# 0xPabloxx/3d-pointcloud-orientation-estimation

Hardware: AMD Instinct MI355X
Metric: clouds/sec fwd+bwd, pointnet_pp_vonMises N=1024 (higher is better)
Workload: dtype f32; 1 GPU; configs[1]: models/pointnet_pp_vonMises.py single-peak KL, N=1024, batch=32 per GPU, fwd+loss+bwd+allreduce+Adam, random-init weights (seed 42), device-side centre sampling; per_gpu_batch=32, global_batch=32, points=1024, parallelism=single, launch=hipGraph(fwd+loss+bwd) + eager all-reduce/Adam (the update clears the gradients)

## Files before the change

### 3d-pointcloud-orientation-estimation_amd/csrc/bn_pool_kernels.hip

```cpp
#include "launch.h"
#include "split_prims.h"

namespace pnpp {

template <int EPB>
__device__ __forceinline__ void slab_reduce_block(const SlabReduceArgs &R, int bid) {
    constexpr int SL = 256 / EPB;
    __shared__ float red[SL][EPB];
    const int total = R.Nc * R.Kvalid;
    const int e = threadIdx.x % EPB, sl = threadIdx.x / EPB;
    const int i = bid * EPB + e;
    float acc = 0.f;
    int c = 0, k = 0;
    if (i < total) {
        c = i / R.Kvalid, k = i - c * R.Kvalid;
        const float *p = R.slab + (size_t)c * R.kp_pad + k;
        const size_t stride = (size_t)R.Nc * R.kp_pad;
        float a0 = 0.f, a1 = 0.f, a2 = 0.f, a3 = 0.f;
        int s = sl;
        for (; s + 3 * SL < R.nsplit; s += 4 * SL) {
            a0 += p[(size_t)s * stride];
            a1 += p[(size_t)(s + SL) * stride];
            a2 += p[(size_t)(s + 2 * SL) * stride];
            a3 += p[(size_t)(s + 3 * SL) * stride];
// ... 631 lines not shown
        ProfScope ps(st, "pool_fwd_merge_kernel G=%d C=%d split=%d", G, C, nsplit);
        hipLaunchKernelGGL(pool_fwd_merge_kernel, dim3((unsigned)cdiv(tot, 256)), dim3(256), 0, st, pmax, parg, G, nsplit, C, out, arg,
                           origin_a, origin_b, norigin);
        PNPP_CHECK_LAUNCH("pool_fwd_merge");
        return PNPP_OK;
    }
    const size_t total = (size_t)G * C;
    const int grid = (int)((total + 255) / 256 < 4096 ? (total + 255) / 256 : 4096);
    ProfScope ps(st, "pool_fwd_kernel G=%d K=%d C=%d", G, K, C);
    hipLaunchKernelGGL(pool_fwd_kernel, dim3(grid), dim3(256), 0, st, z, scale, shift, G, K, C, out, arg, origin_a, origin_b, norigin,
                       zsel);
    PNPP_CHECK_LAUNCH("pool_fwd");
    return PNPP_OK;
}

__device__ __forceinline__ void pool_bwd_block(const float *__restrict__ dout, const int32_t *__restrict__ arg, const float *__restrict__ z,
                                               const float *__restrict__ scale, const float *__restrict__ shift,
                                               const float *__restrict__ mean, const float *__restrict__ istd, int G, int K, int C,
                                               float *__restrict__ dm, double *__restrict__ slab, const float *__restrict__ zsel,
                                               int policy, unsigned bx, unsigned by, unsigned ny) {
    __shared__ double red[4][2][64];
    const int cl = threadIdx.x & 63, gl = threadIdx.x >> 6;
    const int c = bx * 64 + cl;
    double s1 = 0.0, s2 = 0.0;
    if (c < C) {
        const float mu = mean[c], is = istd[c], sc = scale[c], sh = shift[c];
        for (int g = by * 4 + gl; g < G; g += ny * 4) {
            const size_t gi = (size_t)g * C + c;
            const float za = zsel ? zsel[gi] : z[((size_t)g * K + arg[gi]) * C + c];
            const float d = fmaf(za, sc, sh) > 0.f ? dout[gi] : 0.f;
            dm[gi] = d;
            s1 += (double)d;
            s2 += (double)d * (double)((za - mu) * is);
        }
    }
    red[gl][0][cl] = s1;
    red[gl][1][cl] = s2;
    __syncthreads();
    if (gl == 0 && c < C) {
        double a = 0.0, b = 0.0;
#pragma unroll
        for (int i = 0; i < 4; ++i) a += red[i][0][cl], b += red[i][1][cl];
        sp_store(slab + ((size_t)by * 2 + 0) * C + c, a, (policy & ST_STAT_SLABS) != 0);
        sp_store(slab + ((size_t)by * 2 + 1) * C + c, b, (policy & ST_STAT_SLABS) != 0);
    }
}

__global__ void __launch_bounds__(256)
pool_bwd_kernel(const float *__restrict__ dout, const int32_t *__restrict__ arg, const float *__restrict__ z,
                const float *__restrict__ scale, const float *__restrict__ shift, const float *__restrict__ mean,
                const float *__restrict__ istd, int G, int K, int C, float *__restrict__ dm, double *__restrict__ slab,
                const float *__restrict__ zsel, int policy) {
    pool_bwd_block(dout, arg, z, scale, shift, mean, istd, G, K, C, dm, slab, zsel, policy, blockIdx.x, blockIdx.y, gridDim.y);
}

struct PoolBwdArgs {
    const float *dout;
    const int32_t *arg;
    const float *z, *scale, *shift, *mean, *istd;
    int G, K, C;
    float *dm;
    double *slab;
    const float *zsel;
    int policy;
};
template <bool PAIR>
__global__ void __launch_bounds__(256) pool_bwd_ride_kernel(PoolBwdArgs P, int nx, int ny, SlabReduceArgs R1, int n1, SlabReduceArgs R2) {
    const int bid = blockIdx.x, npool = nx * ny;
    if (bid < npool) {
        pool_bwd_block(P.dout, P.arg, P.z, P.scale, P.shift, P.mean, P.istd, P.G, P.K, P.C, P.dm, P.slab, P.zsel, P.policy, bid % nx, bid / nx, ny);
    } else if constexpr (PAIR) {
        if (bid - npool < n1) slab_reduce_block<16>(R1, bid - npool);
        else slab_reduce_block<64>(R2, bid - npool - n1);
    } else {
        slab_reduce_block<64>(R1, bid - npool);
    }
}

int launch_pool_bwd(const float *dout, const int32_t *arg, const float *z, const float *scale, const float *shift,
                    const float *mean, const float *istd, int G, int K, int C, float *dm, double *slab, int *nslab,
                    hipStream_t st, const float *zsel, const SaTail *ride) {
    int gy = cdiv(G, 16);
    if (gy > kMaxStatBlocks) gy = kMaxStatBlocks;
    if (gy < 1) gy = 1;
    *nslab = gy;
    if (ride && ride->kind != PNPP_SA_TAIL_NONE) {
        if (!slab_tail_rides(*ride)) PNPP_TRY(launch_slab_tail(*ride, st));
        else {
            const SlabReduceArgs &R1 = ride->R1, &R2 = ride->R2;
            const PoolBwdArgs P{dout, arg, z, scale, shift, mean, istd, G, K, C, dm, slab, zsel, store_policy()};
            const int nx = cdiv(C, 64), nride = slab_tail_blocks(*ride);
            if (ride->kind == PNPP_SA_TAIL_SLAB_REDUCE2) {
                bool w1, w2;
                int n1, n2;
                slab_reduce2_plan(R1, R2, &w1, &w2, &n1, &n2);
                ProfScope ps(st, "pool_bwd_kernel G=%d K=%d C=%d + slab_reduce2 N=%d K=%d split=%d | N=%d K=%d split=%d", G, K, C, R1.Nc,
                             R1.Kvalid, R1.nsplit, R2.Nc, R2.Kvalid, R2.nsplit);
                hipLaunchKernelGGL(pool_bwd_ride_kernel<true>, dim3(nx * gy + nride), dim3(256), 0, st, P, nx, gy, R1, n1, R2);
            } else {
                ProfScope ps(st, "pool_bwd_kernel G=%d K=%d C=%d + slab_reduce N=%d K=%d split=%d", G, K, C, R1.Nc, R1.Kvalid, R1.nsplit);
                hipLaunchKernelGGL(pool_bwd_ride_kernel<false>, dim3(nx * gy + nride), dim3(256), 0, st, P, nx, gy, R1, 0, R1);
            }
            PNPP_CHECK_LAUNCH("pool_bwd(+tail)");
            return PNPP_OK;
        }
    }
    ProfScope ps(st, "pool_bwd_kernel G=%d K=%d C=%d", G, K, C);
    hipLaunchKernelGGL(pool_bwd_kernel, dim3(cdiv(C, 64), gy), dim3(256), 0, st, dout, arg, z, scale, shift, mean, istd, G, K, C,
                       dm, slab, zsel, store_policy());
    PNPP_CHECK_LAUNCH("pool_bwd");
    return PNPP_OK;
}

int launch_fill_zero(void *p, size_t bytes, hipStream_t st) {
    if (bytes == 0) return PNPP_OK;
    hipError_t e = hipMemsetAsync(p, 0, bytes, st);
    if (e != hipSuccess) {
        set_error("memset failed: %s", hipGetErrorString(e));
        return PNPP_ERR_LAUNCH;
    }
    return PNPP_OK;
}

}
// ... 1 lines not shown
```

### 3d-pointcloud-orientation-estimation_amd/csrc/gemm_wsd3_kernels.hip

```cpp
#include "launch.h"
#include "split_prims.h"

namespace pnpp {

typedef __attribute__((address_space(3))) volatile unsigned wd3_flag;
__device__ int g_wsd3_timeouts;
__device__ __forceinline__ bool wd3_wait(wd3_flag *f, unsigned target) {
    bool ok = true;
    unsigned spins = 0;
    while ((unsigned)__builtin_amdgcn_readfirstlane((int)*f) < target) {
        __builtin_amdgcn_s_sleep(1);
        if (++spins > (1u << 16)) {
            ok = false;
            break;
        }
    }
    asm volatile("" ::: "memory");
    return ok;
}
__device__ __forceinline__ void wd3_post(wd3_flag *f, unsigned v) {
    asm volatile("s_waitcnt lgkmcnt(0)" ::: "memory");
    *f = v;
}

// ... 3 lines not shown
    if (st_on) {                                                       \
        const unsigned long long st_t = __builtin_amdgcn_s_memtime();  \
        st_acc[i] += st_t - st_last;                                   \
        st_last = st_t;                                                \
    }
#else
#define WD3_STAMP(i)
#endif

template <int KD, int BN, bool HANDOFF>
struct Wsd3Lds {
    static constexpr int WPLANE = BN * KD * 2, APLANE = 32 * 128, ABUF = 3 * APLANE, APAIR = 2 * ABUF, BFR = 2 * 3 * 64 * 16;
    static constexpr int OFF_IMG = 3 * WPLANE, OFF_CST = OFF_IMG + 4 * APAIR, OFF_BFR = OFF_CST + 3 * KD * 4;
    static constexpr int OFF_FLG = OFF_BFR + (HANDOFF ? 4 * BFR : 0), END = OFF_FLG + 64;
};

template <int KD, int BN, int AM>
__global__ void __launch_bounds__(512, 1)
gemm_wsd3_kernel(const AOperand A, const float *__restrict__ W, int ldw, int M, int Nout, int ncol, const Epilogue E) {
    constexpr int NC = KD / 64, CT = KD / 32;
    static_assert(BN == 32, "one column tile per workgroup: the consumer wave holds dW (KD x 32) and the dA tile");
    constexpr bool SPLITDW = true;
    constexpr int CTC = SPLITDW ? CT / 2 : CT;
    constexpr bool HANDOFF = KD == 128;
    constexpr bool DW2 = KD == 128 && AM == A_DZ_POOL;
    constexpr bool ACC2 = true;
    constexpr int WPITCH = KD * 2, WPLANE = BN * WPITCH;
    constexpr int APLANE = 32 * 128, ABUF = 3 * APLANE;
    constexpr int APAIR = 2 * ABUF;
    using LY = Wsd3Lds<KD, BN, HANDOFF>;
// ... 70 lines not shown
            d = __builtin_amdgcn_mfma_f32_32x32x16_bf16(al, bh, d, 0, 0, 0);
            d = __builtin_amdgcn_mfma_f32_32x32x16_bf16(ah, bl, d, 0, 0, 0);
            d = __builtin_amdgcn_mfma_f32_32x32x16_bf16(am, bm, d, 0, 0, 0);
            d = __builtin_amdgcn_mfma_f32_32x32x16_bf16(am, bh, d, 0, 0, 0);
            d = __builtin_amdgcn_mfma_f32_32x32x16_bf16(ah, bm, d, 0, 0, 0);
            if constexpr (DW2) {
                dwsm = d;
                dwl = __builtin_amdgcn_mfma_f32_32x32x16_bf16(ah, bh, dwl, 0, 0, 0);
            } else {
                dwl = __builtin_amdgcn_mfma_f32_32x32x16_bf16(ah, bh, d, 0, 0, 0);
            }
        }
    };

    if (tid < 8) ((wd3_flag *)(lds3 + OFF_FLG))[tid] = 0u;
    for (int c = tid; c < KD; c += 512) {
        const float g = A.cst[c], mu = A.cst[A.C + c], is = A.cst[2 * A.C + c], c1 = A.cst[3 * A.C + c], c2 = A.cst[4 * A.C + c];
        const float a = -g * is * c2;
        Tc[c] = g, Tc[KD + c] = a, Tc[2 * KD + c] = -g * c1 - a * mu;
    }
    {
        constexpr int NWF = (KD / 4) * BN / 512;
        f32x4 tw[NWF];
#pragma unroll
        for (int j = 0; j < NWF; ++j) {
            const int f = tid + 512 * j, nl = f % BN, k4 = 4 * (f / BN);
#pragma unroll
            for (int e = 0; e < 4; ++e) tw[j][e] = W[(size_t)(k4 + e) * ldw + n0 + nl];
        }
#pragma unroll
        for (int j = 0; j < NWF; ++j) {
            const int f = tid + 512 * j, nl = f % BN, k4 = 4 * (f / BN);
            uint2 h, m, l;
            sp_split4(tw[j], h, m, l);
            unsigned char *dst = Wp + nl * WPITCH + 16 * ((k4 >> 3) ^ xw(nl)) + 2 * (k4 & 7);
            *reinterpret_cast<uint2 *>(dst) = h;
            *reinterpret_cast<uint2 *>(dst + WPLANE) = m;
            *reinterpret_cast<uint2 *>(dst + 2 * WPLANE) = l;
        }
    }
    __syncthreads();

#ifdef PNPP_STAMPS
    const bool st_on = blockIdx.x == 8 && pair == 0;
    unsigned long long st_acc[8] = {0, 0, 0, 0, 0, 0, 0, 0};
    unsigned long long st_last = __builtin_amdgcn_s_memtime();
#endif
    f32x16 dw[CTC], dws[DW2 ? CTC : 1];
    double s1 = 0.0, s2 = 0.0;
    bool timed_out = false;

    if (producer) {
        const int q = lane & 15, q4 = 4 * q, rb = lane >> 4;
        const __amdgpu_buffer_rsrc_t resZ = sp_buf_rsrc(A.z), resY = sp_buf_rsrc(A.a), resI = sp_buf_rsrc(A.arg);
        const unsigned oa0 = 4u * ((unsigned)rb * (unsigned)KD + (unsigned)q4);
        f32x4 rz[2][8], ry[AM == A_DZ ? 2 : 1][8], rdm[2];
// ... 300 lines not shown

bool wsd3_applies(const AOperand &A, const BOperand &B, int M, int Nout, int Kd, const Epilogue &E) {
    if (!split_products() || matmul_precision() != 0) return false;
    const bool pooled = A.mode == A_DZ_POOL && A.K == 32 && ((Kd == 128 && Nout == 64) || (Kd == 256 && Nout == 128));
    const bool dense = A.mode == A_DZ && Kd == 128 && Nout == 128 && A.a;
    if (M < 8192 || M % 32 != 0 || !(pooled || dense)) return false;
    if (E.mode != E_MASK_STATS || !E.dwslab || E.dw_ld < Nout) return false;
    if (B.trans || B.perm_D >= 0 || (B.rows > 0 && B.rows != Kd) || B.ldb < Nout) return false;
    if (A.lda != Kd || A.C != Kd || E.ldc != Nout) return false;
    if ((((uintptr_t)A.a | (uintptr_t)A.z | (uintptr_t)E.zp | (uintptr_t)E.c | (uintptr_t)A.cst) & 15) != 0) return false;
    if (A.mode == A_DZ_POOL && (((uintptr_t)A.arg) & 15) != 0) return false;
    if ((unsigned long long)M * (unsigned)Kd * 4ull >= 0xfffffff0ull) return false;
    return true;
}

bool try_launch_wsd3(const AOperand &A, const BOperand &B, int M, int Nout, int Kd, const Epilogue &E, int *nslab, hipStream_t st, int *rc,
                     int *dw_slabs) {
    *rc = PNPP_OK;
    if (!dw_slabs || !wsd3_applies(A, B, M, Nout, Kd, E)) return false;
    const int nstrips = M / 32, ncol = Nout / 32;
    const int workers = worker_count(256 / ncol, nstrips, 4);
    if (nslab) *nslab = workers;
    *dw_slabs = workers;
    ProfScope ps(st, "gemm_wsd3_kernel<%d,32,A%d> M=%d N=%d K=%d grid=%dx1", Kd, A.mode, M, Nout, Kd, workers * ncol);
    if (Kd == 256) wsd3_launch<256, 32, A_DZ_POOL>(A, B, M, Nout, E, workers, ncol, st);
    else if (A.mode == A_DZ_POOL) wsd3_launch<128, 32, A_DZ_POOL>(A, B, M, Nout, E, workers, ncol, st);
    else wsd3_launch<128, 32, A_DZ>(A, B, M, Nout, E, workers, ncol, st);
    check_launch("gemm_wsd3", rc);
    return true;
}

#ifdef WD3_PRIO
#define WD3_PRIO_BIT 256u
#else
#define WD3_PRIO_BIT 0u
#endif
unsigned wsd3_build_flags() { return stamps_bit() | WD3_PRIO_BIT; }

int wsd3_timeouts() {
    int v = 0;
    (void)hipMemcpyFromSymbol(&v, HIP_SYMBOL(g_wsd3_timeouts), sizeof(int));
    return v;
}

}

extern "C" int pnpp_debug_wsd3_timeouts(void) { return pnpp::wsd3_timeouts(); }
#ifdef PNPP_STAMPS
extern "C" int pnpp_debug_wsd3_stamps(unsigned long long *out32, int reset) { return pnpp::stamps_io<32>(&pnpp::g_wsd3_stamps, out32, reset); }
#endif
```

### 3d-pointcloud-orientation-estimation_amd/csrc/kernels.h

```cpp
#pragma once
#include "common.h"

namespace pnpp {

int launch_knn(const float *new_xyz, const float *xyz, int B, int S, int N, int k, int32_t *idx, hipStream_t st,
               const int32_t *lengths = nullptr);
int launch_knn_centres(const float *xyz, const int32_t *centre, int B, int S, int N, int k, int32_t *idx, float *out_a,
                       float *out_b, hipStream_t st, const int32_t *lengths = nullptr);
int launch_knn_pair(const float *xyz, int B, int N, const int32_t *centre1, int S1, int k1, int32_t *idx1, float *a1, float *b1,
                    const int32_t *centre2, int S2, int k2, int32_t *idx2, float *a2, float *b2, double *mom, hipStream_t st,
                    const int32_t *lengths = nullptr);
int knn_pair_moment_partials(int B, int S1, int N);
size_t knn_pair_moment_doubles(int B, int S1, int N);
int launch_gather_centres(const float *xyz, const int32_t *centre, int B, int N, int S, float *out_a, float *out_b, hipStream_t st);
int launch_scatter_rows_bwd(const float *dout, const int32_t *idx, int B, int N, int C, int M, float *dpoints, hipStream_t st);

enum AMode {
    A_PLAIN = 0,
    A_BNRELU = 1,
    A_GATHER = 2,
    A_CONCAT = 3,
    A_DZ = 4,
    A_DZ_POOL = 5
};

struct AOperand {
    int mode = A_PLAIN;
    const float *a = nullptr;
    int lda = 0;
    const float *scale = nullptr, *shift = nullptr;
    const float *xyz = nullptr, *new_xyz = nullptr;
    const int32_t *idx = nullptr;
    int D = 0, N = 0, S = 0, K = 0;
    const int32_t *arg = nullptr;
    const float *z = nullptr;
    const float *cst = nullptr;
    int C = 0;
};

enum EMode {
    E_STORE = 0,
    E_STORE_STATS = 1,
    E_MASK_STATS = 2,
    E_BN_APPLY = 3
};

struct BnTail {
    const float *bias = nullptr, *gamma = nullptr, *beta = nullptr;
    float *rm = nullptr, *rv = nullptr;
    long long *nbt = nullptr;
    float momentum = 0.1f, eps = 1e-5f;
    float *mean = nullptr, *istd = nullptr, *scale = nullptr, *shift = nullptr;
// ... 86 lines not shown
bool try_launch_da_dw(const AOperand &dz, const BOperand &W, int M, int Nout, int Kd, const Epilogue &E, int *nslab, const AOperand &a2,
                      int Kp, float *slab, int *nsplit, int *kp_pad, hipStream_t st, int *rc, float *dw_direct = nullptr, int dw_ld = 0);
bool try_launch_mid_gemm(const AOperand &A, const BOperand &B, int M, int Nout, int Kd, const Epilogue &E, int *nslab, hipStream_t st,
                         int *rc);
bool mid_gemm_pools(const AOperand &A, int M, int Nout, int Kd);
bool try_launch_wsf(const AOperand &A, const BOperand &B, int M, int Nout, int Kd, const Epilogue &E, int *nslab, hipStream_t st, int *rc);
bool wsf_applies(const AOperand &A, const BOperand &B, int M, int Nout, int Kd, const Epilogue &E);
int split_products();
void set_split_products(int on);
int store_policy();
void set_store_policy(int mask);
bool try_launch_wsf3(const AOperand &A, const BOperand &B, int M, int Nout, int Kd, const Epilogue &E, int *nslab, hipStream_t st, int *rc);
bool try_launch_wsd3(const AOperand &A, const BOperand &B, int M, int Nout, int Kd, const Epilogue &E, int *nslab, hipStream_t st, int *rc,
                     int *dw_slabs);
int wsd3_timeouts();
bool try_launch_wsp(const AOperand &A, const BOperand &B, int M, int Nout, int Kd, const Epilogue &E, int *nslab, hipStream_t st, int *rc,
                    int *dw_slabs);
bool try_launch_wsq(const AOperand &A, const BOperand &B, int M, int Nout, int Kd, const Epilogue &E, int *nslab, hipStream_t st, int *rc,
                    int *dw_slabs);
bool try_launch_wsx(const AOperand &dz, const BOperand &W, int M, int C1, int C0, const AOperand &geo, const float *W0, int ldw0,
                    const float *scale0, const float *shift0, float *dwslab, double *stat, int *workers_out, hipStream_t st, int *rc);
size_t wsx_stat_doubles();
bool xyz0_applies(int M, int D, int K, int group_all, int L, const int *C);
size_t xyz0_moment_doubles();
int launch_rel_moments(const AOperand &geo, int M, double *mom, int *nmom, hipStream_t st);
int launch_wsf0(const AOperand &geo, int M, const BOperand &W0, const double *mom, int nmom, const BnLayer &bn0, const BnHyper &h,
                const BOperand &W1, const Epilogue &E, int *nslab, hipStream_t st);
int launch_xyz0_post(const SlabReduceArgs &R1, const double *stat, const BOperand &W0, const BnLayer &bn0, double count, int training,
                     float *dW0, int ld0, const BnGrads &g0, hipStream_t st);
int launch_relu_mask(const float *z, const float *scale, const float *shift, size_t n, int C, uint8_t *out, hipStream_t st);
// ... 34 lines not shown
                     hipStream_t st, const DzSide &dz = DzSide());

bool stats_sync_on();
int launch_slab_sum(const double *slab, int nslab, int C, double count, double *glob, double *local, hipStream_t st);
int stats_exchange(const double *slab, int nslab, int C, double count, hipStream_t st, StatsView *out);
int stats_exchange_inplace(int C, hipStream_t st, StatsView *out);
double *stats_buffer_global();
double *stats_buffer_local();

int pool_fwd_splits(int G, int K, int C);
int launch_pool_fwd(const float *z, const float *scale, const float *shift, int G, int K, int C, float *out, int32_t *arg,
                    hipStream_t st, float *origin_a = nullptr, float *origin_b = nullptr, int norigin = 0, void *part = nullptr,
                    float *zsel = nullptr);
int launch_pool_bwd(const float *dout, const int32_t *arg, const float *z, const float *scale, const float *shift,
                    const float *mean, const float *istd, int G, int K, int C, float *dm, double *slab, int *nslab,
                    hipStream_t st, const float *zsel = nullptr, const SaTail *ride = nullptr);

int launch_fill_zero(void *p, size_t bytes, hipStream_t st);

int launch_bn_fold_split(const float *w, int Cin, const float *b, const float *gamma, const float *beta, const float *rm, const float *rv,
                         float eps, int C, int ld, unsigned short *wout, float *bout, hipStream_t st);
int infer_target_wgs();

}
```

### 3d-pointcloud-orientation-estimation_amd/csrc/sa_api.hip

```cpp
#include "launch.h"

namespace pnpp {

struct SaGeom {
    int M, G, maxC;
    int Cin[PNPP_MAX_LAYERS];
    int Kd[PNPP_MAX_LAYERS];
};

static int sa_geom(const pnpp_sa_desc *d, SaGeom *g) {
    PNPP_REQUIRE(d, PNPP_ERR_ARG, "sa: null descriptor");
    PNPP_REQUIRE(d->B > 0 && d->N > 0 && d->S > 0 && d->K > 0 && d->D >= 0, PNPP_ERR_ARG,
                 "sa: bad geometry B=%d N=%d S=%d K=%d D=%d", d->B, d->N, d->S, d->K, d->D);
    PNPP_REQUIRE(d->L >= 1 && d->L <= PNPP_MAX_LAYERS, PNPP_ERR_ARG, "sa: unsupported layer count %d", d->L);
    if (d->group_all) PNPP_REQUIRE(d->S == 1 && d->K == d->N, PNPP_ERR_ARG, "sa: group_all needs S == 1 and K == N");
    PNPP_REQUIRE((long long)d->B * d->S * d->K < (1ll << 31), PNPP_ERR_ARG, "sa: B*S*K overflows int32");
    g->M = d->B * d->S * d->K;
    g->G = d->B * d->S;
    g->maxC = 0;
    for (int l = 0; l < d->L; ++l) {
        PNPP_REQUIRE(d->C[l] > 0 && d->C[l] % 32 == 0, PNPP_ERR_ARG,
                     "sa: mlp channel %d (=%d) must be a positive multiple of 32 for the MFMA path", l, d->C[l]);
        g->maxC = d->C[l] > g->maxC ? d->C[l] : g->maxC;
        g->Cin[l] = l == 0 ? d->D + 3 : d->C[l - 1];
// ... 288 lines not shown
    for (int l = 0; l < d->L; ++l)
        PNPP_REQUIRE(a->conv_w[l] && a->bn_w[l] && a->d_conv_w[l] && a->d_conv_b[l] && a->d_bn_w[l] && a->d_bn_b[l], PNPP_ERR_ARG,
                     "sa_backward: null pointer in layer %d", l);
    L->want_dpoints = d->D > 0 && a->dpoints != nullptr;
    if (L->want_dpoints && d->group_all)
        PNPP_REQUIRE(d->D % 4 == 0, PNPP_ERR_ARG, "sa_backward: feature width D=%d must be a multiple of 4", d->D);
    sa_level_bind(L, const_cast<void *>(a->saved), a->scratch, a->xyz, a->points, a->conv_w, a->bn_w, st);
    for (int l = 0; l < d->L; ++l) L->dbn[l] = BnGrads{a->d_bn_w[l], a->d_bn_b[l], a->d_conv_b[l]};
    return PNPP_OK;
}

struct SaBwdState {
    int cur = 0;
    bool dz_ready = false;
    bool dpoints_done = false;
};

static int sa_bwd_stats(const SaLevel &L, int l, int nslab, StatsView *V) {
    V->slab = L.sc.slab, V->nslab = nslab;
    if (L.d->training) PNPP_TRY(stats_exchange(L.sc.slab, nslab, L.d->C[l], L.count(), L.st, V));
    return PNPP_OK;
}

static bool tail_clear_of(const SaTail &T, const SaScratch &sc) {
    auto hits = [&](const SlabReduceArgs &R) {
        const char *lo = (const char *)R.slab, *hi = lo + (size_t)R.nsplit * R.Nc * R.kp_pad * sizeof(float);
        auto over = [&](const void *b, const void *e) { return lo < (const char *)e && (const char *)b < hi; };
        return over(sc.slab, sc.dy[0]) || over(sc.dm, sc.cst);
    };
    return !(hits(T.R1) || (T.kind == PNPP_SA_TAIL_SLAB_REDUCE2 && hits(T.R2)));
}
// ... 9 lines not shown
    AOperand dz_top = L.dz_operand(Lm, 0);
    S->dz_ready = L.small;
    if (pooled_src) {
        if (L.ride) PNPP_TRY(launch_slab_tail(*L.ride, L.st));
        dz_top.a = a->dout;
        PooledSource ps;
        ps.dout = a->dout, ps.zsel = sv.zmax, ps.scale = sv.scale[Lm], ps.shift = sv.shift[Lm], ps.G = g.G;
        return launch_bn_finalize_bwd(StatsView(), L.count(), d->training, L.bn[Lm], sc.cst, L.dbn[Lm], L.st, L.dz_side(&dz_top), &ps);
    }
    int nslab = 0;
    const SaTail *ride = L.ride;
    if (ride && !tail_clear_of(*ride, sc)) {
        PNPP_TRY(launch_slab_tail(*ride, L.st));
        ride = nullptr;
    }
    PNPP_TRY(launch_pool_bwd(a->dout, sv.arg, sv.z[Lm], sv.scale[Lm], sv.shift[Lm], sv.mean[Lm], sv.istd[Lm], g.G, d->K, d->C[Lm], sc.dm,
                             sc.slab, &nslab, L.st, L.keeps_zmax ? sv.zmax : nullptr, ride));
    StatsView V;
    PNPP_TRY(sa_bwd_stats(L, Lm, nslab, &V));
    return launch_bn_finalize_bwd(V, L.count(), d->training, L.bn[Lm], sc.cst, L.dbn[Lm], L.st, L.dz_side(&dz_top));
}

static int sa_bwd_tail(const SaLevel &L, const SaTail &T) {
    if (!L.defer) return launch_slab_tail(T, L.st);
    *L.defer = T;
    return PNPP_OK;
}

static int sa_bwd_dz(const SaLevel &L, int l, SaBwdState *S, AOperand *dz) {
    *dz = L.dz_operand(l, S->cur);
    if (!L.small) return PNPP_OK;
    if (!S->dz_ready) PNPP_TRY(launch_dz_materialize(*dz, L.g.M, L.d->C[l], L.sc.dzbuf, L.st));
    S->dz_ready = false;
    *dz = AOperand();
    dz->mode = A_PLAIN, dz->a = L.sc.dzbuf, dz->lda = L.d->C[l];
    return PNPP_OK;
}

static int sa_bwd_xyz0_tail(const SaLevel &L, const pnpp_sa_bwd_args *a, const AOperand &dz) {
    const pnpp_sa_desc *d = L.d;
    const SaGeom &g = L.g;
    int workers = 0, rc = PNPP_OK, C = d->C[1];
    const bool taken = try_launch_wsx(dz, L.weight(1, C), g.M, C, d->C[0], L.layer0_operand(), L.conv_w[0], g.Cin[0], L.sv.scale[0],
                                      L.sv.shift[0], L.sc.dwslab, L.sc.slab, &workers, L.st, &rc);
    PNPP_REQUIRE(taken, PNPP_ERR_ARG, "sa_backward: the coordinate-level backward kernel does not take this call (alignment?)");
// ... 30 lines not shown
    return PNPP_OK;
}

static int sa_bwd_layer(const SaLevel &L, const pnpp_sa_bwd_args *a, int l, const AOperand &dz, SaBwdState *S) {
    const pnpp_sa_desc *d = L.d;
    const SaGeom &g = L.g;
    const SaSaved &sv = L.sv;
    const SaScratch &sc = L.sc;
    const int C = d->C[l];
    const AOperand a2 = L.input_of(l);
    int nsplit, kp_pad;
    dw_plan(g.M, C, g.Cin[l], &nsplit, &kp_pad);
    int fused_slabs = 0, nslab_next = 0;
    bool pair_done = false;
    if (l > 0) {
        Epilogue E;
        E.mode = E_MASK_STATS;
        E.c = sc.dy[S->cur ^ 1], E.ldc = d->C[l - 1], E.slab = sc.slab, E.zp = sv.z[l - 1];
        E.scale = sv.scale[l - 1], E.shift = sv.shift[l - 1], E.mu = sv.mean[l - 1], E.istd = sv.istd[l - 1];
        E.dwslab = sc.dwslab, E.dw_ld = d->C[l - 1];
        const BOperand W = L.weight(l, C);
        int rc = PNPP_OK;
        pair_done = try_launch_da_dw(dz, W, g.M, d->C[l - 1], C, E, &nslab_next, a2, g.Cin[l], sc.dwslab, &nsplit, &kp_pad, L.st, &rc,
                                     a->d_conv_w[l], g.Cin[l]);
        if (pair_done) PNPP_TRY(rc);
        else PNPP_TRY(launch_gemm(dz, W, g.M, d->C[l - 1], C, E, &nslab_next, L.st, &fused_slabs));
    }
    const bool xyz_only = l == 0 && d->D == 0 && (a2.mode == A_GATHER || (a2.mode == A_CONCAT && g.M >= 8192)) &&
                          dw_xyz_splits(g.M) <= nsplit * (kp_pad / 4);
    if (xyz_only) {
        PNPP_TRY(launch_dw_xyz(dz, C, a2, g.M, sc.dwslab, L.st));
        nsplit = dw_xyz_splits(g.M), kp_pad = 4;
    } else if (fused_slabs == 0 && !pair_done) {
        if (l == 0 && L.want_dpoints && d->group_all) {
            int rc = PNPP_OK;
// ... 149 lines not shown
```

### 3d-pointcloud-orientation-estimation_amd/pnpp_hip/_lib.py

```python
from __future__ import annotations

import ctypes as C
import os

HERE = os.path.dirname(os.path.abspath(__file__))
LIB_PATH = os.path.join(HERE, "libpnpp_hip.so")

PNPP_MAX_LAYERS = 4
PNPP_OK, PNPP_ERR_ARG, PNPP_ERR_RANGE, PNPP_ERR_LAUNCH, PNPP_ERR_WORKSPACE = 0, -1, -2, -3, -4
NORM_NONE, NORM_BATCH, NORM_LAYER = 0, 1, 2

_fp = C.c_void_p


class SaDesc(C.Structure):
    _fields_ = [("B", C.c_int), ("N", C.c_int), ("S", C.c_int), ("K", C.c_int), ("D", C.c_int), ("L", C.c_int),
                ("C", C.c_int * PNPP_MAX_LAYERS), ("group_all", C.c_int), ("training", C.c_int),
                ("eps", C.c_float), ("momentum", C.c_float)]


_PL = _fp * PNPP_MAX_LAYERS


class SaFwdArgs(C.Structure):
# ... 226 lines not shown
    "pnpp_mean_points": (_i, [_fp, _i, _i, _i, _fp, _fp]),
    "pnpp_linear_smallk_bwd_scratch_bytes": (_sz, [_i, _i]),
    "pnpp_linear_smallk_bwd": (_i, [_fp, _fp, _i, _i, _i, _fp, _fp, _fp, _fp]),
    "pnpp_attention_bwd": (_i, [_fp, _fp, _fp, _fp, _i, _i, _i, _i, _i, _fp, _fp, _f, _fp, _fp, _fp]),
    "pnpp_add_layernorm_bwd_scratch_bytes": (_sz, [_i, _i]),
    "pnpp_add_layernorm_bwd": (_i, [_fp, _fp, _fp, _fp, _i, _i, _f, _fp, _fp, _fp, _fp]),
    "pnpp_mean_points_bwd": (_i, [_fp, _i, _i, _i, _fp, _fp]),
    "pnpp_set_matmul_precision": (_i, [_i]),
    "pnpp_set_stats_exchange": (_i, [STATS_EXCHANGE_FN, C.c_void_p, C.c_void_p, _sz]),
    "pnpp_stats_exchange_enabled": (_i, []),
    "pnpp_get_matmul_precision": (_i, []),
    "pnpp_set_split_products": (_i, [_i]),
    "pnpp_get_split_products": (_i, []),
    "pnpp_set_store_policy": (_i, [_i]),
    "pnpp_get_store_policy": (_i, []),
    "pnpp_adam_step": (_i, [_fp, _fp, _fp, _fp, _sz, _i, _f, _f, _f, _f, _f, _fp]),
    "pnpp_adam_step_zero": (_i, [_fp, _fp, _fp, _fp, _sz, _i, _f, _f, _f, _f, _f, _fp]),
    "pnpp_adam_step_dev": (_i, [_fp, _fp, _fp, _fp, _sz, _fp, _f, _f, _f, _f, _f, _i, _fp]),
    "pnpp_adam_step_clip": (_i, [_fp, _fp, _fp, _fp, _sz, _i, _f, _f, _f, _f, _f, _fp, _f, _i, _fp]),
    "pnpp_adam_step_dev_clip": (_i, [_fp, _fp, _fp, _fp, _sz, _fp, _f, _f, _f, _f, _f, _fp, _f, _i, _fp]),
    "pnpp_sumsq": (_i, [_fp, _sz, _fp, _fp, _sz, _fp]),
    "pnpp_adamw_step": (_i, [C.POINTER(OptimDesc), _fp, _fp, _fp, _fp, _fp, _sz, _fp, _fp, _fp]),
    "pnpp_lr_factor": (_i, [C.POINTER(OptimDesc), _u64, C.POINTER(C.c_double)]),
    "pnpp_pn_pool_saved_bytes": (_sz, [C.POINTER(PnPoolDesc)]),
    "pnpp_pn_pool_scratch_bytes": (_sz, [C.POINTER(PnPoolDesc)]),
    "pnpp_pn_pool_forward": (_i, [C.POINTER(PnPoolDesc), C.POINTER(PnPoolFwdArgs), _fp]),
    "pnpp_pn_pool_backward": (_i, [C.POINTER(PnPoolDesc), C.POINTER(PnPoolBwdArgs), _fp]),
    "pnpp_pn_pool_saved_route": (_fp, [C.POINTER(PnPoolDesc), _fp]),
    "pnpp_pn_pool_saved_zsel": (_fp, [C.POINTER(PnPoolDesc), _fp]),
    "pnpp_pn_pool_saved_ypre": (_fp, [C.POINTER(PnPoolDesc), _fp]),
# ... 31 lines not shown
    if _lib is None:
        if not os.path.exists(LIB_PATH):
            raise HipExtensionMissing(
                f"{LIB_PATH} is missing: build it with `python -m pnpp_hip.build` (hipcc, gfx950). "
                "This package has no CPU or PyTorch fallback.")
        try:
            h = C.CDLL(LIB_PATH)
        except OSError as e:
            raise HipExtensionMissing(f"cannot load {LIB_PATH}: {e}") from e
        for name, (res, args) in SIGNATURES.items():
            fn = getattr(h, name)
            fn.restype = res
            fn.argtypes = args
        if h.pnpp_abi_version() != 5:
            raise HipExtensionMissing("libpnpp_hip.so ABI version mismatch; rebuild it")
        _lib = h
    return _lib


def last_error() -> str:
    return lib().pnpp_last_error().decode("utf-8", "replace")


def check(rc: int) -> None:
    if rc == PNPP_OK:
        return
    msg = last_error()
    if rc == PNPP_ERR_ARG:
        raise ValueError(msg)
    raise RuntimeError(msg)
# ... 1 lines not shown
```

### 3d-pointcloud-orientation-estimation_amd/pnpp_hip/ops.py

```python
from __future__ import annotations

import ctypes as C
import os
from typing import Optional, Sequence, Tuple

import torch

from . import _lib as L
from .lengths import fps_starts, packed_lengths, ragged_lengths


def _stream() -> int:
    return torch.cuda.current_stream().cuda_stream


def _need_gpu(t: torch.Tensor, name: str) -> None:
    if not isinstance(t, torch.Tensor):
        raise TypeError(f"{name} must be a torch.Tensor")
    if not t.is_cuda:
        raise RuntimeError(f"{name} is on '{t.device}': the pnpp HIP operators run on an AMD GPU only "
                           "(no CPU fallback exists in this package)")


def _f32(t: torch.Tensor, name: str) -> torch.Tensor:
# ... 101 lines not shown


def get_float32_products() -> str:
    return "split" if L.lib().pnpp_get_split_products() else "mfma"


STORE_DW_SLABS, STORE_STAT_SLABS, STORE_STREAMS = 1, 2, 4


def set_store_policy(mask: int) -> None:
    L.check(L.lib().pnpp_set_store_policy(int(mask)))


def get_store_policy() -> int:
    return L.lib().pnpp_get_store_policy()


def square_distance(src: torch.Tensor, dst: torch.Tensor) -> torch.Tensor:
    src, dst = _f32(src, "src"), _f32(dst, "dst")
    B, S, _ = src.shape
    N = dst.shape[1]
    out = torch.empty(B, S, N, device=src.device, dtype=torch.float32)
    L.check(L.lib().pnpp_square_distance(src.data_ptr(), dst.data_ptr(), B, S, N, out.data_ptr(), _stream()))
    return out


def knn(new_xyz: torch.Tensor, xyz: torch.Tensor, k: int, lengths=None) -> torch.Tensor:
    new_xyz, xyz = _f32(new_xyz, "new_xyz"), _f32(xyz, "xyz")
    B, S, _ = new_xyz.shape
    N = xyz.shape[1]
# ... 1445 lines not shown
```

### include/pnpp_hip.h

```cpp
#ifndef PNPP_HIP_H
#define PNPP_HIP_H

#include <stddef.h>
#include <stdint.h>

#ifdef __cplusplus
extern "C" {
#endif

typedef enum {
    PNPP_OK = 0,
    PNPP_ERR_ARG = -1,
    PNPP_ERR_RANGE = -2,
    PNPP_ERR_LAUNCH = -3,
    PNPP_ERR_WORKSPACE = -4
} pnpp_status;

const char *pnpp_last_error(void);
int pnpp_abi_version(void);

int pnpp_profile_enable(int on);
int pnpp_profile_report(char *buf_host, size_t buflen);


// ... 237 lines not shown
                       void *stream);
size_t pnpp_add_layernorm_bwd_scratch_bytes(int M, int E);
int pnpp_add_layernorm_bwd(const float *x, const float *r, const float *w, const float *dy, int M, int E, float eps,
                           float *du, float *dwb, void *scratch, void *stream);
int pnpp_mean_points_bwd(const float *dy, int B, int N, int E, float *dx, void *stream);

int pnpp_set_matmul_precision(int bf16_operands);
int pnpp_get_matmul_precision(void);

int pnpp_set_split_products(int on);
int pnpp_get_split_products(void);

int pnpp_set_store_policy(int mask);
int pnpp_get_store_policy(void);
int pnpp_debug_wsd3_timeouts(void);

typedef int (*pnpp_stats_exchange_fn)(double *buf, size_t n_doubles, void *stream, void *user);
int pnpp_set_stats_exchange(pnpp_stats_exchange_fn fn, void *user, double *buf, size_t buf_doubles);
int pnpp_stats_exchange_enabled(void);

typedef struct {
    int B, N;
    int K, C;
    int relu;
    int training;
    float eps, momentum;
} pnpp_pn_pool_desc;

typedef struct {
    const float *a;
// ... 250 lines not shown
```

Baseline: 60780 clouds/s.

## Fuse BatchNorm-backward stat finish into the wsd3 dz GEMM prologue

When the top SA level's dz GEMM runs through the wsd3 kernel, the pool backward now writes a bounded number of per-slab partial sums. The GEMM prologue then reduces those slabs and computes the BN-backward constants and dgamma/dbeta/dbias itself, which removes the separate stats-finish kernel launch. To keep the slab count small, pool backward gains a narrow variant with 16 channels per block and batched, unrolled loads. The trade is extra prologue work and LDS staging inside the GEMM, and redundant reduction in every block.

```diff
diff --git a/3d-pointcloud-orientation-estimation_amd/csrc/bn_pool_kernels.hip b/3d-pointcloud-orientation-estimation_amd/csrc/bn_pool_kernels.hip
--- a/3d-pointcloud-orientation-estimation_amd/csrc/bn_pool_kernels.hip
+++ b/3d-pointcloud-orientation-estimation_amd/csrc/bn_pool_kernels.hip
@@ -669,24 +669,52 @@
     return PNPP_OK;
 }
 
+constexpr int kPoolNarrow = 16;
+template <int CB = 64>
 __device__ __forceinline__ void pool_bwd_block(const float *__restrict__ dout, const int32_t *__restrict__ arg, const float *__restrict__ z,
                                                const float *__restrict__ scale, const float *__restrict__ shift,
                                                const float *__restrict__ mean, const float *__restrict__ istd, int G, int K, int C,
                                                float *__restrict__ dm, double *__restrict__ slab, const float *__restrict__ zsel,
                                                int policy, unsigned bx, unsigned by, unsigned ny) {
-    __shared__ double red[4][2][64];
-    const int cl = threadIdx.x & 63, gl = threadIdx.x >> 6;
-    const int c = bx * 64 + cl;
+    constexpr int GL = 256 / CB;
+    __shared__ double red[GL][2][CB];
+    const int cl = threadIdx.x % CB, gl = threadIdx.x / CB;
+    const int c = bx * CB + cl;
     double s1 = 0.0, s2 = 0.0;
     if (c < C) {
         const float mu = mean[c], is = istd[c], sc = scale[c], sh = shift[c];
-        for (int g = by * 4 + gl; g < G; g += ny * 4) {
-            const size_t gi = (size_t)g * C + c;
-            const float za = zsel ? zsel[gi] : z[((size_t)g * K + arg[gi]) * C + c];
-            const float d = fmaf(za, sc, sh) > 0.f ? dout[gi] : 0.f;
+        auto pre_bn = [&](int g, size_t gi) { return zsel ? zsel[gi] : z[((size_t)g * K + arg[gi]) * C + c]; };
+        auto take = [&](size_t gi, float za, float dv) {
+            const float d = fmaf(za, sc, sh) > 0.f ? dv : 0.f;
             dm[gi] = d;
             s1 += (double)d;
             s2 += (double)d * (double)((za - mu) * is);
+        };
+        if constexpr (CB == 64) {
+            for (int g = by * GL + gl; g < G; g += ny * GL) {
+                const size_t gi = (size_t)g * C + c;
+                const float za = pre_bn(g, gi);
+                take(gi, za, dout[gi]);
+            }
+        } else {
+            const int step = ny * GL;
+            auto batches = [&](auto n_c) {
+                constexpr int N = decltype(n_c)::value;
+                for (int g0 = by * GL + gl; g0 < G; g0 += N * step) {
+                    float za[N], dv[N];
+#pragma unroll
+                    for (int j = 0; j < N; ++j) {
+                        const int g = min(g0 + j * step, G - 1);
+                        const size_t gi = (size_t)g * C + c;
+                        za[j] = pre_bn(g, gi), dv[j] = dout[gi];
+                    }
+#pragma unroll
+                    for (int j = 0; j < N; ++j)
+                        if (g0 + j * step < G) take((size_t)(g0 + j * step) * C + c, za[j], dv[j]);
+                }
+            };
+            if (G > 4 * step) batches(std::integral_constant<int, 8>{});
+            else batches(std::integral_constant<int, 4>{});
         }
     }
     red[gl][0][cl] = s1;
@@ -695,18 +723,19 @@
     if (gl == 0 && c < C) {
         double a = 0.0, b = 0.0;
 #pragma unroll
-        for (int i = 0; i < 4; ++i) a += red[i][0][cl], b += red[i][1][cl];
+        for (int i = 0; i < GL; ++i) a += red[i][0][cl], b += red[i][1][cl];
         sp_store(slab + ((size_t)by * 2 + 0) * C + c, a, (policy & ST_STAT_SLABS) != 0);
         sp_store(slab + ((size_t)by * 2 + 1) * C + c, b, (policy & ST_STAT_SLABS) != 0);
     }
 }
 
+template <int CB>
 __global__ void __launch_bounds__(256)
 pool_bwd_kernel(const float *__restrict__ dout, const int32_t *__restrict__ arg, const float *__restrict__ z,
                 const float *__restrict__ scale, const float *__restrict__ shift, const float *__restrict__ mean,
                 const float *__restrict__ istd, int G, int K, int C, float *__restrict__ dm, double *__restrict__ slab,
                 const float *__restrict__ zsel, int policy) {
-    pool_bwd_block(dout, arg, z, scale, shift, mean, istd, G, K, C, dm, slab, zsel, policy, blockIdx.x, blockIdx.y, gridDim.y);
+    pool_bwd_block<CB>(dout, arg, z, scale, shift, mean, istd, G, K, C, dm, slab, zsel, policy, blockIdx.x, blockIdx.y, gridDim.y);
 }
 
 struct PoolBwdArgs {
@@ -719,11 +748,11 @@
     const float *zsel;
     int policy;
 };
-template <bool PAIR>
+template <bool PAIR, int CB>
 __global__ void __launch_bounds__(256) pool_bwd_ride_kernel(PoolBwdArgs P, int nx, int ny, SlabReduceArgs R1, int n1, SlabReduceArgs R2) {
     const int bid = blockIdx.x, npool = nx * ny;
     if (bid < npool) {
-        pool_bwd_block(P.dout, P.arg, P.z, P.scale, P.shift, P.mean, P.istd, P.G, P.K, P.C, P.dm, P.slab, P.zsel, P.policy, bid % nx, bid / nx, ny);
+        pool_bwd_block<CB>(P.dout, P.arg, P.z, P.scale, P.shift, P.mean, P.istd, P.G, P.K, P.C, P.dm, P.slab, P.zsel, P.policy, bid % nx, bid / nx, ny);
     } else if constexpr (PAIR) {
         if (bid - npool < n1) slab_reduce_block<16>(R1, bid - npool);
         else slab_reduce_block<64>(R2, bid - npool - n1);
@@ -734,9 +763,11 @@
 
 int launch_pool_bwd(const float *dout, const int32_t *arg, const float *z, const float *scale, const float *shift,
                     const float *mean, const float *istd, int G, int K, int C, float *dm, double *slab, int *nslab,
-                    hipStream_t st, const float *zsel, const SaTail *ride) {
+                    hipStream_t st, const float *zsel, const SaTail *ride, int max_slabs) {
+    const bool narrow = max_slabs > 0;
+    const int cb = narrow ? kPoolNarrow : 64, most = narrow ? max_slabs : kMaxStatBlocks;
     int gy = cdiv(G, 16);
-    if (gy > kMaxStatBlocks) gy = kMaxStatBlocks;
+    if (gy > most) gy = most;
     if (gy < 1) gy = 1;
     *nslab = gy;
     if (ride && ride->kind != PNPP_SA_TAIL_NONE) {
@@ -744,25 +775,29 @@
         else {
             const SlabReduceArgs &R1 = ride->R1, &R2 = ride->R2;
             const PoolBwdArgs P{dout, arg, z, scale, shift, mean, istd, G, K, C, dm, slab, zsel, store_policy()};
-            const int nx = cdiv(C, 64), nride = slab_tail_blocks(*ride);
+            const int nx = cdiv(C, cb), nride = slab_tail_blocks(*ride);
             if (ride->kind == PNPP_SA_TAIL_SLAB_REDUCE2) {
                 bool w1, w2;
                 int n1, n2;
                 slab_reduce2_plan(R1, R2, &w1, &w2, &n1, &n2);
                 ProfScope ps(st, "pool_bwd_kernel G=%d K=%d C=%d + slab_reduce2 N=%d K=%d split=%d | N=%d K=%d split=%d", G, K, C, R1.Nc,
                              R1.Kvalid, R1.nsplit, R2.Nc, R2.Kvalid, R2.nsplit);
-                hipLaunchKernelGGL(pool_bwd_ride_kernel<true>, dim3(nx * gy + nride), dim3(256), 0, st, P, nx, gy, R1, n1, R2);
+                if (narrow) hipLaunchKernelGGL((pool_bwd_ride_kernel<true, kPoolNarrow>), dim3(nx * gy + nride), dim3(256), 0, st, P, nx, gy, R1, n1, R2);
+                else hipLaunchKernelGGL((pool_bwd_ride_kernel<true, 64>), dim3(nx * gy + nride), dim3(256), 0, st, P, nx, gy, R1, n1, R2);
             } else {
                 ProfScope ps(st, "pool_bwd_kernel G=%d K=%d C=%d + slab_reduce N=%d K=%d split=%d", G, K, C, R1.Nc, R1.Kvalid, R1.nsplit);
-                hipLaunchKernelGGL(pool_bwd_ride_kernel<false>, dim3(nx * gy + nride), dim3(256), 0, st, P, nx, gy, R1, 0, R1);
+                if (narrow) hipLaunchKernelGGL((pool_bwd_ride_kernel<false, kPoolNarrow>), dim3(nx * gy + nride), dim3(256), 0, st, P, nx, gy, R1, 0, R1);
+                else hipLaunchKernelGGL((pool_bwd_ride_kernel<false, 64>), dim3(nx * gy + nride), dim3(256), 0, st, P, nx, gy, R1, 0, R1);
             }
             PNPP_CHECK_LAUNCH("pool_bwd(+tail)");
             return PNPP_OK;
         }
     }
     ProfScope ps(st, "pool_bwd_kernel G=%d K=%d C=%d", G, K, C);
-    hipLaunchKernelGGL(pool_bwd_kernel, dim3(cdiv(C, 64), gy), dim3(256), 0, st, dout, arg, z, scale, shift, mean, istd, G, K, C,
-                       dm, slab, zsel, store_policy());
+    if (narrow) hipLaunchKernelGGL(pool_bwd_kernel<kPoolNarrow>, dim3(cdiv(C, kPoolNarrow), gy), dim3(256), 0, st, dout, arg, z, scale, shift, mean, istd, G, K, C,
+                                   dm, slab, zsel, store_policy());
+    else hipLaunchKernelGGL(pool_bwd_kernel<64>, dim3(cdiv(C, 64), gy), dim3(256), 0, st, dout, arg, z, scale, shift, mean, istd, G, K, C,
+                            dm, slab, zsel, store_policy());
     PNPP_CHECK_LAUNCH("pool_bwd");
     return PNPP_OK;
 }
diff --git a/3d-pointcloud-orientation-estimation_amd/csrc/gemm_wsd3_kernels.hip b/3d-pointcloud-orientation-estimation_amd/csrc/gemm_wsd3_kernels.hip
--- a/3d-pointcloud-orientation-estimation_amd/csrc/gemm_wsd3_kernels.hip
+++ b/3d-pointcloud-orientation-estimation_amd/csrc/gemm_wsd3_kernels.hip
@@ -41,6 +41,8 @@
     static constexpr int OFF_IMG = 3 * WPLANE, OFF_CST = OFF_IMG + 4 * APAIR, OFF_BFR = OFF_CST + 3 * KD * 4;
     static constexpr int OFF_FLG = OFF_BFR + (HANDOFF ? 4 * BFR : 0), END = OFF_FLG + 64;
 };
+
+constexpr int WSD3_FIN_BYTES = 64 * 1024;
 
 template <int KD, int BN, int AM>
 __global__ void __launch_bounds__(512, 1)
@@ -141,10 +143,32 @@
     };
 
     if (tid < 8) ((wd3_flag *)(lds3 + OFF_FLG))[tid] = 0u;
-    for (int c = tid; c < KD; c += 512) {
-        const float g = A.cst[c], mu = A.cst[A.C + c], is = A.cst[2 * A.C + c], c1 = A.cst[3 * A.C + c], c2 = A.cst[4 * A.C + c];
-        const float a = -g * is * c2;
-        Tc[c] = g, Tc[KD + c] = a, Tc[2 * KD + c] = -g * c1 - a * mu;
+    constexpr int FIN_P = 512 / (2 * KD), FIN_LD = WSD3_FIN_BYTES / (2 * KD * 8) / FIN_P;
+    const bool fin = AM == A_DZ_POOL && A.fin.slab != nullptr;
+    double *fin_stage = reinterpret_cast<double *>(lds3 + OFF_IMG);
+    static_assert(FIN_P * 2 * KD * 8 <= 4 * APAIR, "the staged parts fit the chunk images");
+    float fin_g = 1.f, fin_mu = 0.f, fin_is = 0.f;
+    double fin_v[FIN_LD];
+    if constexpr (AM == A_DZ_POOL) {
+        if (fin) {
+            if (tid < KD) {
+                if (A.fin.gamma) fin_g = A.fin.gamma[tid];
+                fin_mu = A.fin.mean[tid], fin_is = A.fin.istd[tid];
+            }
+            const int j = tid % (2 * KD), p = tid / (2 * KD);
+#pragma unroll
+            for (int i = 0; i < FIN_LD; ++i) {
+                const int s = p + FIN_P * i;
+                fin_v[i] = A.fin.slab[(size_t)min(s, A.fin.nslab - 1) * (2 * KD) + j];
+            }
+        }
+    }
+    if (!fin) {
+        for (int c = tid; c < KD; c += 512) {
+            const float g = A.cst[c], mu = A.cst[A.C + c], is = A.cst[2 * A.C + c], c1 = A.cst[3 * A.C + c], c2 = A.cst[4 * A.C + c];
+            const float a = -g * is * c2;
+            Tc[c] = g, Tc[KD + c] = a, Tc[2 * KD + c] = -g * c1 - a * mu;
+        }
     }
     {
         constexpr int NWF = (KD / 4) * BN / 512;
@@ -154,6 +178,14 @@
             const int f = tid + 512 * j, nl = f % BN, k4 = 4 * (f / BN);
 #pragma unroll
             for (int e = 0; e < 4; ++e) tw[j][e] = W[(size_t)(k4 + e) * ldw + n0 + nl];
+        }
+        if constexpr (AM == A_DZ_POOL) {
+            if (fin) {
+                double acc = 0.0;
+#pragma unroll
+                for (int i = 0; i < FIN_LD; ++i) acc += tid / (2 * KD) + FIN_P * i < A.fin.nslab ? fin_v[i] : 0.0;
+                fin_stage[tid] = acc;
+            }
         }
 #pragma unroll
         for (int j = 0; j < NWF; ++j) {
@@ -167,6 +199,28 @@
         }
     }
     __syncthreads();
+    if constexpr (AM == A_DZ_POOL) {
+        if (fin) {
+            if (tid < KD) {
+                const int c = tid;
+                double s1 = fin_stage[c], s2 = fin_stage[KD + c];
+#pragma unroll
+                for (int p = 1; p < FIN_P; ++p) s1 += fin_stage[p * 2 * KD + c], s2 += fin_stage[p * 2 * KD + KD + c];
+                const float g = fin_g * fin_is;
+                const float c1 = A.fin.training ? (float)(s1 / A.fin.count) : 0.f, c2 = A.fin.training ? (float)(s2 / A.fin.count) : 0.f;
+                const float a = -g * fin_is * c2;
+                Tc[c] = g, Tc[KD + c] = a, Tc[2 * KD + c] = -g * c1 - a * fin_mu;
+                if (worker == 0 && col_blk == 0) {
+                    float *cst = A.fin.cst;
+                    cst[c] = g, cst[KD + c] = fin_mu, cst[2 * KD + c] = fin_is, cst[3 * KD + c] = c1, cst[4 * KD + c] = c2;
+                    if (A.fin.dgamma) A.fin.dgamma[c] = (float)s2;
+                    if (A.fin.dbeta) A.fin.dbeta[c] = (float)s1;
+                    if (A.fin.dbias) A.fin.dbias[c] = A.fin.training ? 0.f : (float)((double)g * s1);
+                }
+            }
+            __syncthreads();
+        }
+    }
 
 #ifdef PNPP_STAMPS
     const bool st_on = blockIdx.x == 8 && pair == 0;
@@ -497,15 +551,30 @@
     return true;
 }
 
+static int g_fin_fusion = 1;
+static bool fin_fusion_on() { return g_fin_fusion != 0; }
+
+int wsd3_fin_slabs(int C) { return WSD3_FIN_BYTES / (2 * C * (int)sizeof(double)); }
+
+bool wsd3_finishes(const AOperand &A, const BOperand &B, int M, int Nout, int Kd, const Epilogue &E) {
+    return fin_fusion_on() && !stats_sync_on() && A.mode == A_DZ_POOL && wsd3_applies(A, B, M, Nout, Kd, E);
+}
+
 bool try_launch_wsd3(const AOperand &A, const BOperand &B, int M, int Nout, int Kd, const Epilogue &E, int *nslab, hipStream_t st, int *rc,
                      int *dw_slabs) {
     *rc = PNPP_OK;
+    const bool fin = A.fin.slab != nullptr;
+    if (fin && !(dw_slabs && wsd3_finishes(A, B, M, Nout, Kd, E) && A.fin.nslab >= 1 && A.fin.nslab <= wsd3_fin_slabs(Kd) && A.fin.cst)) {
+        set_error("gemm_wsd3: asked to finish the BatchNorm-backward sums of a launch it does not take (nslab=%d)", A.fin.nslab);
+        *rc = PNPP_ERR_ARG;
+        return true;
+    }
     if (!dw_slabs || !wsd3_applies(A, B, M, Nout, Kd, E)) return false;
     const int nstrips = M / 32, ncol = Nout / 32;
     const int workers = worker_count(256 / ncol, nstrips, 4);
     if (nslab) *nslab = workers;
     *dw_slabs = workers;
-    ProfScope ps(st, "gemm_wsd3_kernel<%d,32,A%d> M=%d N=%d K=%d grid=%dx1", Kd, A.mode, M, Nout, Kd, workers * ncol);
+    ProfScope ps(st, "gemm_wsd3_kernel<%d,32,A%d> M=%d N=%d K=%d grid=%dx1%s", Kd, A.mode, M, Nout, Kd, workers * ncol, fin ? " +fin" : "");
     if (Kd == 256) wsd3_launch<256, 32, A_DZ_POOL>(A, B, M, Nout, E, workers, ncol, st);
     else if (A.mode == A_DZ_POOL) wsd3_launch<128, 32, A_DZ_POOL>(A, B, M, Nout, E, workers, ncol, st);
     else wsd3_launch<128, 32, A_DZ>(A, B, M, Nout, E, workers, ncol, st);
@@ -529,6 +598,11 @@
 }
 
 extern "C" int pnpp_debug_wsd3_timeouts(void) { return pnpp::wsd3_timeouts(); }
+extern "C" int pnpp_set_fin_fusion(int on) {
+    pnpp::g_fin_fusion = on != 0;
+    return PNPP_OK;
+}
+extern "C" int pnpp_get_fin_fusion(void) { return pnpp::g_fin_fusion; }
 #ifdef PNPP_STAMPS
 extern "C" int pnpp_debug_wsd3_stamps(unsigned long long *out32, int reset) { return pnpp::stamps_io<32>(&pnpp::g_wsd3_stamps, out32, reset); }
 #endif
diff --git a/3d-pointcloud-orientation-estimation_amd/csrc/kernels.h b/3d-pointcloud-orientation-estimation_amd/csrc/kernels.h
--- a/3d-pointcloud-orientation-estimation_amd/csrc/kernels.h
+++ b/3d-pointcloud-orientation-estimation_amd/csrc/kernels.h
@@ -22,6 +22,14 @@
     A_CONCAT = 3,
     A_DZ = 4,
     A_DZ_POOL = 5
+};
+
+struct DzFinish {
+    const double *slab = nullptr;
+    int nslab = 0, training = 0;
+    double count = 0.0;
+    const float *gamma = nullptr, *mean = nullptr, *istd = nullptr;
+    float *cst = nullptr, *dgamma = nullptr, *dbeta = nullptr, *dbias = nullptr;
 };
 
 struct AOperand {
@@ -36,6 +44,7 @@
     const float *z = nullptr;
     const float *cst = nullptr;
     int C = 0;
+    DzFinish fin;
 };
 
 enum EMode {
@@ -152,6 +161,8 @@
 bool try_launch_wsd3(const AOperand &A, const BOperand &B, int M, int Nout, int Kd, const Epilogue &E, int *nslab, hipStream_t st, int *rc,
                      int *dw_slabs);
 int wsd3_timeouts();
+bool wsd3_finishes(const AOperand &A, const BOperand &B, int M, int Nout, int Kd, const Epilogue &E);
+int wsd3_fin_slabs(int C);
 bool try_launch_wsp(const AOperand &A, const BOperand &B, int M, int Nout, int Kd, const Epilogue &E, int *nslab, hipStream_t st, int *rc,
                     int *dw_slabs);
 bool try_launch_wsq(const AOperand &A, const BOperand &B, int M, int Nout, int Kd, const Epilogue &E, int *nslab, hipStream_t st, int *rc,
@@ -216,7 +227,7 @@
                     float *zsel = nullptr);
 int launch_pool_bwd(const float *dout, const int32_t *arg, const float *z, const float *scale, const float *shift,
                     const float *mean, const float *istd, int G, int K, int C, float *dm, double *slab, int *nslab,
-                    hipStream_t st, const float *zsel = nullptr, const SaTail *ride = nullptr);
+                    hipStream_t st, const float *zsel = nullptr, const SaTail *ride = nullptr, int max_slabs = 0);
 
 int launch_fill_zero(void *p, size_t bytes, hipStream_t st);
 
diff --git a/3d-pointcloud-orientation-estimation_amd/csrc/sa_api.hip b/3d-pointcloud-orientation-estimation_amd/csrc/sa_api.hip
--- a/3d-pointcloud-orientation-estimation_amd/csrc/sa_api.hip
+++ b/3d-pointcloud-orientation-estimation_amd/csrc/sa_api.hip
@@ -326,7 +326,20 @@
     int cur = 0;
     bool dz_ready = false;
     bool dpoints_done = false;
+    DzFinish fin;
 };
+
+static Epilogue sa_bwd_da_epilogue(const SaLevel &L, int l, int cur) {
+    const pnpp_sa_desc *d = L.d;
+    const SaSaved &sv = L.sv;
+    const SaScratch &sc = L.sc;
+    Epilogue E;
+    E.mode = E_MASK_STATS;
+    E.c = sc.dy[cur ^ 1], E.ldc = d->C[l - 1], E.slab = sc.slab, E.zp = sv.z[l - 1];
+    E.scale = sv.scale[l - 1], E.shift = sv.shift[l - 1], E.mu = sv.mean[l - 1], E.istd = sv.istd[l - 1];
+    E.dwslab = sc.dwslab, E.dw_ld = d->C[l - 1];
+    return E;
+}
 
 static int sa_bwd_stats(const SaLevel &L, int l, int nslab, StatsView *V) {
     V->slab = L.sc.slab, V->nslab = nslab;
@@ -366,6 +379,16 @@
         PNPP_TRY(launch_slab_tail(*ride, L.st));
         ride = nullptr;
     }
+    if (Lm > 0 && !L.small &&
+        wsd3_finishes(dz_top, L.weight(Lm, d->C[Lm]), g.M, d->C[Lm - 1], d->C[Lm], sa_bwd_da_epilogue(L, Lm, S->cur))) {
+        double *slab = sc.slab + (size_t)kMaxStatBlocks * g.maxC;
+        PNPP_TRY(launch_pool_bwd(a->dout, sv.arg, sv.z[Lm], sv.scale[Lm], sv.shift[Lm], sv.mean[Lm], sv.istd[Lm], g.G, d->K, d->C[Lm], sc.dm,
+                                 slab, &nslab, L.st, L.keeps_zmax ? sv.zmax : nullptr, ride, wsd3_fin_slabs(d->C[Lm])));
+        const BnLayer &bn = L.bn[Lm];
+        const BnGrads &gr = L.dbn[Lm];
+        S->fin = DzFinish{slab, nslab, d->training, L.count(), bn.gamma, bn.mean, bn.istd, sc.cst, gr.dgamma, gr.dbeta, gr.dbias};
+        return PNPP_OK;
+    }
     PNPP_TRY(launch_pool_bwd(a->dout, sv.arg, sv.z[Lm], sv.scale[Lm], sv.shift[Lm], sv.mean[Lm], sv.istd[Lm], g.G, d->K, d->C[Lm], sc.dm,
                              sc.slab, &nslab, L.st, L.keeps_zmax ? sv.zmax : nullptr, ride));
     StatsView V;
@@ -381,6 +404,7 @@
 
 static int sa_bwd_dz(const SaLevel &L, int l, SaBwdState *S, AOperand *dz) {
     *dz = L.dz_operand(l, S->cur);
+    if (l == L.d->L - 1) dz->fin = S->fin;
     if (!L.small) return PNPP_OK;
     if (!S->dz_ready) PNPP_TRY(launch_dz_materialize(*dz, L.g.M, L.d->C[l], L.sc.dzbuf, L.st));
     S->dz_ready = false;
@@ -441,11 +465,7 @@
     int fused_slabs = 0, nslab_next = 0;
     bool pair_done = false;
     if (l > 0) {
-        Epilogue E;
-        E.mode = E_MASK_STATS;
-        E.c = sc.dy[S->cur ^ 1], E.ldc = d->C[l - 1], E.slab = sc.slab, E.zp = sv.z[l - 1];
-        E.scale = sv.scale[l - 1], E.shift = sv.shift[l - 1], E.mu = sv.mean[l - 1], E.istd = sv.istd[l - 1];
-        E.dwslab = sc.dwslab, E.dw_ld = d->C[l - 1];
+        const Epilogue E = sa_bwd_da_epilogue(L, l, S->cur);
         const BOperand W = L.weight(l, C);
         int rc = PNPP_OK;
         pair_done = try_launch_da_dw(dz, W, g.M, d->C[l - 1], C, E, &nslab_next, a2, g.Cin[l], sc.dwslab, &nsplit, &kp_pad, L.st, &rc,
diff --git a/3d-pointcloud-orientation-estimation_amd/pnpp_hip/_lib.py b/3d-pointcloud-orientation-estimation_amd/pnpp_hip/_lib.py
--- a/3d-pointcloud-orientation-estimation_amd/pnpp_hip/_lib.py
+++ b/3d-pointcloud-orientation-estimation_amd/pnpp_hip/_lib.py
@@ -264,6 +264,8 @@
     "pnpp_get_split_products": (_i, []),
     "pnpp_set_store_policy": (_i, [_i]),
     "pnpp_get_store_policy": (_i, []),
+    "pnpp_set_fin_fusion": (_i, [_i]),
+    "pnpp_get_fin_fusion": (_i, []),
     "pnpp_adam_step": (_i, [_fp, _fp, _fp, _fp, _sz, _i, _f, _f, _f, _f, _f, _fp]),
     "pnpp_adam_step_zero": (_i, [_fp, _fp, _fp, _fp, _sz, _i, _f, _f, _f, _f, _f, _fp]),
     "pnpp_adam_step_dev": (_i, [_fp, _fp, _fp, _fp, _sz, _fp, _f, _f, _f, _f, _f, _i, _fp]),
@@ -325,6 +327,8 @@
             fn.argtypes = args
         if h.pnpp_abi_version() != 5:
             raise HipExtensionMissing("libpnpp_hip.so ABI version mismatch; rebuild it")
+        if os.environ.get("PNPP_NO_FIN_FUSION", "0") not in ("", "0"):
+            h.pnpp_set_fin_fusion(0)
         _lib = h
     return _lib
 
diff --git a/3d-pointcloud-orientation-estimation_amd/pnpp_hip/ops.py b/3d-pointcloud-orientation-estimation_amd/pnpp_hip/ops.py
--- a/3d-pointcloud-orientation-estimation_amd/pnpp_hip/ops.py
+++ b/3d-pointcloud-orientation-estimation_amd/pnpp_hip/ops.py
@@ -139,6 +139,14 @@
 
 def get_store_policy() -> int:
     return L.lib().pnpp_get_store_policy()
+
+
+def set_fin_fusion(on: bool) -> None:
+    L.check(L.lib().pnpp_set_fin_fusion(1 if on else 0))
+
+
+def get_fin_fusion() -> bool:
+    return bool(L.lib().pnpp_get_fin_fusion())
 
 
 def square_distance(src: torch.Tensor, dst: torch.Tensor) -> torch.Tensor:
diff --git a/include/pnpp_hip.h b/include/pnpp_hip.h
--- a/include/pnpp_hip.h
+++ b/include/pnpp_hip.h
@@ -275,6 +275,8 @@
 int pnpp_set_store_policy(int mask);
 int pnpp_get_store_policy(void);
 int pnpp_debug_wsd3_timeouts(void);
+int pnpp_set_fin_fusion(int on);
+int pnpp_get_fin_fusion(void);
 
 typedef int (*pnpp_stats_exchange_fn)(double *buf, size_t n_doubles, void *stream, void *user);
 int pnpp_set_stats_exchange(pnpp_stats_exchange_fn fn, void *user, double *buf, size_t buf_doubles);
```

Result: no change. 61310 clouds/s (median of 6 runs) (+0.9%).
